# benedikthoward/ENPH459-Super-Resolution

Measured on AMD Instinct MI355X. Metric: HR megapixels/sec at x4 upscale (SAA + 80-iteration IBP reconstruction), higher is better.
Workload: dtype f32; 1 GPU; C2: x4 multi-frame SR of 64x64 LR patches -> 256x256 HR, N=16 frames (all 4x4 sub-pixel phases), 7x7 Gaussian PSF, shift_and_add + ibp(80 it, step 0.5); patches_per_gpu=1024, global_patches=1024, factor=4, frames=16, n_iter=80, parallelism=patch-sharded x1, no collective

## Files before the change

### enph459-super-resolution_amd/csrc/srx_dtile.hpp

```cpp
#pragma once
#include "srx_patch.hpp"

namespace srx {
namespace dtile {

using patch::AxisC;
using patch::AxisW;
using patch::f8;
using patch::FIX;
using patch::ld4;
using patch::ld_u2;
using patch::NN_PAD;
using patch::RW;
using patch::sload8;
using patch::SLOT0;
using patch::SLOT1;
using patch::st4;
using patch::u32x4;
using patch::YW;

constexpr int RY = 256;
constexpr int HL = 32;
constexpr int ALIGN_Y = 4, ALIGN_X = 16;

template <int NSX> struct Lds {
    static constexpr int NW = 4 * NSX;
    static constexpr int OFF_YT = NW * RW, OFF_YL = OFF_YT + 4 * YW, OFF_GT = OFF_YL + 4 * YW, OFF_GL = OFF_GT + 3 * YW,
                         OFF_ROW = OFF_GL + 3 * YW, OFF_PART = OFF_ROW + 256, WORDS = OFF_PART + 2 * NW + 2;
    static_assert(WORDS * 4 <= 160 * 1024, "LDS budget");
};

struct TileD {
    int oy, ox;
    int y0, y1, x0, x1;
    int ntab;
    int flags;
};

struct DArgs {
    int H, W, tiles_x, tiles_y;
    AxisC y, x;
    int ngrp, c01;
    float sn;
};

struct DTabs {
    const float *Mt;
    const unsigned *Mt8;
    const int *m8;
    const float *Ct;
    const AxisW *aw;
    const TileD *tiles;
    const unsigned long long *rowm, *colm;
    const int *nn;
    const uint2 *nrec;
    const uint2 *nent;
    const float2 *Mn;
    int ntabs;
    const float *k2;
};

struct AxisTiles {
    int n;
    int o[64], a[65];
};

static inline bool plan_axis_tiles(int L, int RL, int align, AxisTiles &at)
{
    if (L < RL || L % align)
// ... 270 lines not shown
#pragma unroll
            for (int i = 0; i < NW; i++)
                t += part[i];
            err_prev[(size_t)b * err_stride] = (t + Vtot[b]) * scale;
        }
        __syncthreads();
    }
    const int sq0 = ((td.oy + 64 * s) >> 2) * W * 16;
    const int tb0 = (((td.ox + 64 * u) >> 2) * H + td.oy + 64 * s) * 16;
    const int m80 = (((td.ox + 64 * u) >> 4) * H + td.oy + 64 * s) * 16;
    auto uniform64 = [](unsigned long long v) {
        return (unsigned long long)(unsigned)__builtin_amdgcn_readfirstlane((int)(unsigned)v) |
               (unsigned long long)(unsigned)__builtin_amdgcn_readfirstlane((int)(unsigned)(v >> 32)) << 32;
    };
    const unsigned long long rmask = C01 ? uniform64(tb.rowm[(size_t)((td.flags >> 8) & 0xfff) * 4 + s]) : 0ull;
    const unsigned long long cmask = C01 ? uniform64(tb.colm[(size_t)((td.flags >> 20) & 0xfff) * 4 + u]) : 0ull;

#define SRX_DT_LOCALS()                                              \
    int tid = tid0;                                                  \
    asm volatile("" : "+v"(tid));                                    \
    const int lane = tid & 63;                                       \
    int sql = sq0, tbl = tb0, m8l = m80;                             \
    asm volatile("" : "+s"(sql), "+s"(tbl), "+s"(m8l));              \
    const int vcol = (td.ox + 64 * u + lane) * 16;                   \
    (void)tbl, (void)m8l, (void)sql, (void)vcol

    float a[64], r[64];
    float yex = 0.f;
    {
        SRX_DT_LOCALS();
#pragma unroll
        for (int q = 0; q < 16; q++)
            ld4(rs_src, vcol, sql + q * W * 16, a[4 * q], a[4 * q + 1], a[4 * q + 2], a[4 * q + 3]);
        if (PSF == 0) {
            patch::blur_block(a, s == 0, s == 3, Rown, Rup, Rdn, SLOT0, lane, sload8(awy));
        } else {
            Rown[SLOT0 + lane] = a[0];
            Rown[SLOT0 + 64 + lane] = a[1];
            Rown[SLOT0 + 128 + lane] = a[2];
            Rown[SLOT0 + 192 + lane] = a[61];
            Rown[SLOT0 + 256 + lane] = a[62];
            Rown[SLOT0 + 320 + lane] = a[63];
            __syncthreads();
            float hl[3] = {0.f, 0.f, 0.f}, hr[3] = {0.f, 0.f, 0.f};
            if (s != 0)
                hl[0] = Rup[SLOT0 + 192 + lane], hl[1] = Rup[SLOT0 + 256 + lane], hl[2] = Rup[SLOT0 + 320 + lane];
            if (s != 3)
                hr[0] = Rdn[SLOT0 + lane], hr[1] = Rdn[SLOT0 + 64 + lane], hr[2] = Rdn[SLOT0 + 128 + lane];
            patch::blur2d_pass1<PSF == 2 ? 2 : 3>(a, hl, hr, Rown, lane, tb.k2);
            __syncthreads();
            patch::blur2d_fix<PSF == 2 ? 2 : 3>(a, u == 0, u == NSX - 1, Rown, Rlf, Rrt, lane, [](int) {}, [](int, float v) { return v; });
        }
        __builtin_amdgcn_sched_barrier(0);
        patch::fwd_chain(a, s == 0, s == 3, Rown, Rup, Rdn, SLOT1, SLOT0, lane, sload8(awy + 16), yex);
        __builtin_amdgcn_sched_barrier(0);
        if (exy && s == 0)
            rowbuf[64 * u + lane] = yex;
        __syncthreads();
        if (exy && s == 3)
            a[63] = rowbuf[64 * u + lane];
        __builtin_amdgcn_sched_barrier(0);
        patch::transpose64(a, r, Rown, lane);
        __builtin_amdgcn_sched_barrier(0);
    }
    float sq = 0.f;
    {
        SRX_DT_LOCALS();
        const bool wrapped = exy && s == 3 && lane == 63;
        const int gy = wrapped ? -1 : 64 * s + lane;
        const bool rownear = wrapped || gy < nby;
        const bool rowown = !wrapped && gy >= td.y0 && gy < td.y1;
        const float crow = C01 ? (float)((rmask >> lane) & 1ull) : 0.f;
        if (PSF == 0)
            patch::blur_block(r, u == 0, u == NSX - 1, Rown, Rlf, Rrt, SLOT0, lane, sload8(awx));
        __builtin_amdgcn_sched_barrier(0);
        float yexx = 0.f;
        patch::fwd_chain(r, u == 0, u == NSX - 1, Rown, Rlf, Rrt, SLOT1, SLOT0, lane, sload8(awx + 16), yexx);
        __builtin_amdgcn_sched_barrier(0);
        const __amdgpu_buffer_rsrc_t rsNe = fused::plane_rsrc(tb.nent, (size_t)da.ngrp * tb.ntabs * NN_PAD);
        const int tab0 = max(td.ntab, 0) * NN_PAD;
        if (nn > 0) {
            const __amdgpu_buffer_rsrc_t rsNr = fused::plane_rsrc(tb.nrec + tab0, (size_t)nn);
            const __amdgpu_buffer_rsrc_t rsMn = fused::plane_rsrc(tb.Mn + ((size_t)b * tb.ntabs) * NN_PAD + tab0, (size_t)nn);
            uint2 nr[NPT], ne[NPT];
            float2 nm[NPT];
#pragma unroll
            for (int i = 0; i < NPT; i++) {
                const int t8 = (tid + i * NTHR) * 8;
                nr[i] = ld_u2(rsNr, t8), ne[i] = ld_u2(rsNe, tab0 * 8 + t8);
                const uint2 m = ld_u2(rsMn, t8);
                nm[i] = make_float2(__uint_as_float(m.x), __uint_as_float(m.y));
            }
            {
                const bool toprow = wrapped || (s == 0 && lane <= nby);
                if (toprow) {
                    float *dst = Yt + (gy + exy) * YW + 64 * u + exx;
#pragma unroll
                    for (int j = 0; j < 64; j++)
                        dst[j] = r[j];
                    if (u == 0 && exx)
                        dst[-1] = yexx;
                }
                if (left && u == 0) {
                    float *dst = Yl + (gy + exy) * 4 + exx;
#pragma unroll
                    for (int j = 0; j < 3; j++)
                        if (j <= nbx)
                            dst[j] = r[j];
                    if (exx)
                        dst[-1] = yexx;
                }
            }
            __syncthreads();
#pragma unroll
            for (int i = 0; i < NPT; i++) {
                const int t = tid + i * NTHR;
                if (t < nn) {
                    const int cnt = nr[i].x & 255, cu = (nr[i].x >> 8) & 255, dst = nr[i].x >> 16;
                    float ys = (cnt > 0 ? Ystrip[ne[i].x & 0xffff] : 0.f) + (cnt > 1 ? Ystrip[ne[i].x >> 16] : 0.f) +
                               (cnt > 2 ? Ystrip[ne[i].y & 0xffff] : 0.f) + (cnt > 3 ? Ystrip[ne[i].y >> 16] : 0.f);
                    for (int g = 1; 4 * g < cnt; g++) {
                        const uint2 e = ld_u2(rsNe, ((g * tb.ntabs) * NN_PAD + tab0 + t) * 8);
                        const int c = cnt - 4 * g;
                        ys += (c > 0 ? Ystrip[e.x & 0xffff] : 0.f) + (c > 1 ? Ystrip[e.x >> 16] : 0.f) + (c > 2 ? Ystrip[e.y & 0xffff] : 0.f) +
                              (c > 3 ? Ystrip[e.y >> 16] : 0.f);
                    }
                    Gstrip[dst] = nm[i].x - ys;
                    if (cu > 0) {
                        const float gu = nm[i].y - (float)cu * Ystrip[nr[i].y];
                        sq += gu * gu / (float)cu;
// ... 113 lines not shown
            sq += (rownear || !rowown) ? 0.f : sqf;
            if ((top && s == 0) || (exy && s == 3)) {
                const float *src = Gt + (rownear ? gy + exy : 0) * YW + 64 * u + exx;
#pragma unroll
                for (int j0 = 0; j0 < 64; j0 += 8) {
                    float v[8];
                    int o = j0;
                    asm volatile("" : "+v"(o), "+v"(r[j0 > 0 ? j0 - 1 : 0])::"memory");
#pragma unroll
                    for (int j = 0; j < 8; j++)
                        v[j] = src[o + j];
#pragma unroll
                    for (int j = 0; j < 8; j++) {
                        r[j0 + j] = rownear ? v[j] : r[j0 + j];
                        asm volatile("" : "+v"(r[j0 + j]));
                    }
                    __builtin_amdgcn_sched_barrier(0);
                }
                if (u == 0 && exx && rownear)
                    gexx = src[-1];
            }
            if (left && u == 0 && !rownear) {
                const float *src = Gl + (gy - nby) * 3 + exx;
#pragma unroll
                for (int j = 0; j < 3; j++)
                    if (j < nbx)
                        r[j] = src[j];
                if (exx)
                    gexx = src[-1];
            }
        }
        if (epart) {
            const double ws = wave_sum((double)sq);
            if (lane == 0)
                part[wave] = ws;
        }
        __builtin_amdgcn_sched_barrier(0);
        {
            Rown[SLOT1 + lane] = r[0];
            Rown[SLOT1 + 64 + lane] = r[1];
            Rown[SLOT1 + 128 + lane] = r[63];
            __syncthreads();
            if (epart && tid == 0) {
                double t = 0.0;
#pragma unroll
                for (int i = 0; i < NW; i++)
                    t += part[i];
                epart[(size_t)b * gridDim.x + wid] = t;
            }
            const float gtop = exx ? gexx : r[0];
            const float gm1 = u == 0 ? gtop : Rlf[SLOT1 + 128 + lane];
            const float gp1 = u == NSX - 1 ? 0.f : Rrt[SLOT1 + lane], gp2 = u == NSX - 1 ? 0.f : Rrt[SLOT1 + 64 + lane];
            float hlo[3], hhi[3];
            patch::bwd_chain_x<PSF == 0>(r, a, u == 0, u == NSX - 1, Rown, Rlf, Rrt, SLOT0 + 384, SLOT0, lane, sload8(awx + 16), sload8(awx + 8), gm1, gp1, gp2, gtop,
                                         [](int) {}, [](int, float v) { return v; }, hlo, hhi);
        }
        __builtin_amdgcn_sched_barrier(0);
        __syncthreads();
        __builtin_amdgcn_sched_barrier(0);
        patch::transpose64(a, r, Rown, lane);
        __builtin_amdgcn_sched_barrier(0);
    }
    {
        SRX_DT_LOCALS();
        float hv[16], hw[16];
        if (exy && s == 3) {
            rowbuf[64 * u + lane] = r[63];
            r[63] = 0.f;
        }
        Rown[SLOT0 + lane] = r[0];
        Rown[SLOT0 + 64 + lane] = r[1];
        Rown[SLOT0 + 128 + lane] = r[63];
        __syncthreads();
        const float gtop = exy ? rowbuf[64 * u + lane] : r[0];
        const float gm1 = s == 0 ? gtop : Rup[SLOT0 + 128 + lane];
        const float gp1 = s == 3 ? 0.f : Rdn[SLOT0 + lane], gp2 = s == 3 ? 0.f : Rdn[SLOT0 + 64 + lane];
        float dep = 0.f;
        auto mid = [&](int q) {
                             auto load16 = [&](float(&ld)[16], int bq) {
                                 int so = sq0;
                                 asm volatile("" : "+s"(so), "+v"(dep)::"memory");
#pragma unroll
                                 for (int k = 0; k < 4; k++)
                                     ld4(rs_src, vcol, so + (4 * bq + k) * W * 16, ld[4 * k], ld[4 * k + 1], ld[4 * k + 2], ld[4 * k + 3]);
                             };
                             if (q == 0)
                                 load16(hv, 0), load16(hw, 1);
                             if (q == 1)
                                 load16(hv, 2);
                             else if (q == 2)
                                 load16(hw, 3);
                         };
        auto post = [&](int i, float corr) {
                             const float v = __builtin_amdgcn_fmed3f(fmaf(corr, sn, ((i >> 4) & 1) ? hw[i & 15] : hv[i & 15]), 0.f, 255.f);
                             if ((i & 15) == 15)
                                 dep = v;
                             return v;
                         };
        if (PSF == 0) {
            patch::bwd_chain(r, a, s == 0, s == 3, Rown, Rup, Rdn, SLOT1 + 384, SLOT1, lane, sload8(awy + 16), sload8(awy + 8), gm1, gp1, gp2, gtop, mid, post);
        } else {
            float hl[3], hr[3];
            patch::bwd_chain_x<false>(r, a, s == 0, s == 3, Rown, Rup, Rdn, SLOT1 + 384, SLOT1, lane, sload8(awy + 16), sload8(awy + 8), gm1, gp1, gp2, gtop, [](int) {},
                                      [](int, float v) { return v; }, hl, hr);
            patch::blur2d_pass1<PSF == 2 ? 2 : 3>(a, hl, hr, Rown, lane, tb.k2 + 56);
            __syncthreads();
            patch::blur2d_fix<PSF == 2 ? 2 : 3>(a, u == 0, u == NSX - 1, Rown, Rlf, Rrt, lane, mid, post);
        }
        __builtin_amdgcn_sched_barrier(0);
        const int cc = 64 * u + lane;
        const int vst = (cc >= td.x0 && cc < td.x1) ? vcol : 0x7ffffff0;
#pragma unroll
        for (int q = 0; q < 16; q++) {
            const int rw = 64 * s + 4 * q;
            if (rw >= td.y0 && rw < td.y1)
                st4(rs_dst, vst, sql + q * W * 16, a[4 * q], a[4 * q + 1], a[4 * q + 2], a[4 * q + 3]);
        }
    }
#undef SRX_DT_LOCALS
}

template <bool C01, int NSX, int PSF = 0>
__global__ void __launch_bounds__(256 * NSX)
    k_ibp_dtile(const float *__restrict__ hr_src, float *__restrict__ hr_dst, DTabs tb, DArgs da, double *__restrict__ epart,
                const double *__restrict__ eprev, const double *__restrict__ Vtot, double scale, double *__restrict__ err_prev, int err_stride)
{
    __shared__ float lds[Lds<NSX>::WORDS];
    if (__builtin_amdgcn_readfirstlane(tb.m8[blockIdx.y]) != 0)
        dtile_body<C01, true, NSX, PSF>(lds, hr_src, hr_dst, tb, da, epart, eprev, Vtot, scale, err_prev, err_stride);
    else
        dtile_body<C01, false, NSX, PSF>(lds, hr_src, hr_dst, tb, da, epart, eprev, Vtot, scale, err_prev, err_stride);
}

static inline size_t tabs_bytes(int B, int N, int H, int W)
{
    const size_t ngrp = ((size_t)N + 3) / 4, plane = (size_t)H * W, ntabs = 128, ntiles = 1024;
    return 3 * align_up((size_t)B * plane * 4) + align_up((size_t)B * (W / 4) * H * 4) + align_up((size_t)B * 4) + align_up(plane * 4) +
           align_up(2 * sizeof(AxisW)) + align_up(ntiles * sizeof(TileD)) + 2 * align_up(64 * 4 * 8) + align_up(ntabs * 4) +
           align_up(ntabs * NN_PAD * 8) + align_up(ngrp * ntabs * NN_PAD * 8) + align_up((size_t)B * ntabs * NN_PAD * 8) +
           2 * align_up((size_t)B * ntiles * 8) + align_up(112 * 4);
}

struct FrameN {
    int n[SRX_MAX_FRAMES];
};
__global__ void __launch_bounds__(256)
    k_dtile_setup(AxisTiles ty, AxisTiles tx, FrameN ny, FrameN nx, int N, int f, int H, int W, int nsx, TileD *__restrict__ tiles,
                  unsigned long long *__restrict__ rowm, unsigned long long *__restrict__ colm)
{
    const int tid = blockIdx.x * 256 + threadIdx.x;
    for (int i = tid; i < ty.n * tx.n; i += gridDim.x * 256) {
        const int y = i / tx.n, x = i - y * tx.n;
        TileD t;
        t.oy = ty.o[y], t.ox = tx.o[x];
        t.y0 = ty.a[y] - t.oy, t.y1 = ty.a[y + 1] - t.oy, t.x0 = tx.a[x] - t.ox, t.x1 = tx.a[x + 1] - t.ox;
        t.flags = (y == 0 ? 1 : 0) | (x == 0 ? 2 : 0) | y << 8 | x << 20;
// ... 137 lines not shown
```

### enph459-super-resolution_amd/csrc/srx_patch.hpp

```cpp
#pragma once
#include "srx_mosaic.hpp"

namespace srx {
namespace patch {

#ifndef SRX_PARK16
#define SRX_PARK16 1
#endif
#ifndef SRX_ADDTID
#define SRX_ADDTID 1
#endif
#ifndef SRX_M0_NOP
#define SRX_M0_NOP "s_nop 0\n\t"
#endif
#ifndef SRX_TRANSPOSE_DEF
#define SRX_TRANSPOSE_DEF 1
#endif
#ifndef SRX_PATCH_DBG
#define SRX_PATCH_DBG 0
#endif
constexpr int PN = 256;
constexpr int TSD = 66;
constexpr int RW = 32 * TSD;
constexpr int SLOT0 = 0, SLOT1 = 1024;
constexpr int FIX = 16;
constexpr int YW = 260;
constexpr int OFF_YT = 16 * RW, OFF_YL = OFF_YT + 4 * YW, OFF_GT = OFF_YL + 4 * YW, OFF_GL = OFF_GT + 3 * YW,
              OFF_ROW = OFF_GL + 3 * YW, OFF_PART = OFF_ROW + PN, LDS_WORDS = OFF_PART + 32;
static_assert(LDS_WORDS * 4 <= 160 * 1024, "LDS budget");

constexpr double ZD = -0.26794919243112270647;
constexpr float PZ = (float)ZD;
constexpr float K2 = (float)(1.0 / (1.0 - ZD));
constexpr float K1 = (float)(1.0 / ((1.0 - ZD) * (1.0 - ZD)));
constexpr float K3 = (float)(ZD / (1.0 - ZD * ZD));
constexpr float K4 = (float)(1.0 / (1.0 - ZD * ZD));
struct ZPow {
    float v[FIX];
    constexpr ZPow() : v()
    {
        double p = ZD;
        for (int i = 0; i < FIX; i++) {
            v[i] = (float)p;
            p *= ZD;
        }
    }
};
__device__ constexpr ZPow ZP{};

typedef float f8 __attribute__((ext_vector_type(8)));
struct AxisW {
    float kb[8];
    float kt[8];
    float wfb[8];
};
struct AxisC {
    int ex;
    int nb;
    int E;
};
__device__ __forceinline__ f8 sload8(const float *p)
{
    f8 v;
    asm volatile("s_load_dwordx8 %0, %1, 0x0\n\ts_waitcnt lgkmcnt(0)" : "=s"(v) : "s"(p) : "memory");
    return v;
}

constexpr int NN_PAD = 2048;

struct PatchArgs {
    AxisC y, x;
    int nn, ntop;
    int ngrp;
    int c01;
    unsigned long long ry[4], rx[4];
    float sn;
};

struct PatchTabs {
    const float *Mt;
    const unsigned *Mt8;
    const int *m8;
    const float *Ct;
    const AxisW *aw;
    const uint2 *nrec;
    const uint2 *nent;
    const float2 *Mn;
    const float *k2;
};

static inline bool axis_ok(const mosaic::AxisPlan &pl, int N, int f)
{
    int nmin = pl.n[0], nmax = pl.n[0];
    for (int k = 1; k < N; k++)
        nmin = std::min(nmin, pl.n[k]), nmax = std::max(nmax, pl.n[k]);
    return !pl.zero && nmax >= 0 && nmax <= 1 && nmin <= 0 && nmax - nmin <= 3 && nmax - nmin <= f - 1 && -nmin < f;
}

static inline bool eligible(int elem_bytes, int N, int H, int W, const double *sh, const double *k, int kh, int kw, int f, bool rank1_only)
{
    if (elem_bytes != 4 || H != PN || W != PN || f < 2)
// ... 294 lines not shown
                asm volatile("" : "=v"(r[j]));
        }
        if ((lane >> 5) == h) {
#else
        if (h == 0 || (lane >> 5) == h) {
#endif
            const float2 *row = reinterpret_cast<const float2 *>(Tw + (lane & 31) * TSD);
#pragma unroll
            for (int k = 0; k < 32; k++) {
                const float2 v = row[k];
                r[2 * k] = v.x, r[2 * k + 1] = v.y;
            }
        }
        __builtin_amdgcn_wave_barrier();
    }
}

#ifndef SRX_CHAIN_NSUB
#define SRX_CHAIN_NSUB 2
#endif
template <bool REV> __device__ __forceinline__ void chain64(float (&a)[64], float st0)
{
    constexpr int NSUB = SRX_CHAIN_NSUB, L = 64 / NSUB;
    static_assert(NSUB == 1 || L >= FIX, "a fix-up may not reach into the next sub-chain's start");
    const float z = PZ;
    auto at = [&](int i) -> float & { return a[REV ? 63 - i : i]; };
    float st[NSUB];
#pragma unroll
    for (int k = 0; k < NSUB; k++)
        st[k] = k == 0 ? st0 : 0.f;
#pragma unroll
    for (int i = 0; i < L; i++) {
#pragma unroll
        for (int k = 0; k < NSUB; k++) {
            st[k] = fmaf(z, st[k], at(k * L + i));
            at(k * L + i) = st[k];
        }
    }
    if (NSUB > 1) {
        float e[NSUB];
        e[0] = st[0];
#pragma unroll
        for (int k = 1; k < NSUB; k++)
            e[k] = L == FIX ? fmaf(ZP.v[FIX - 1], e[k - 1], st[k]) : st[k];
#pragma unroll
        for (int k = 1; k < NSUB; k++) {
#pragma unroll
            for (int i = 0; i < FIX; i++)
                at(k * L + i) = fmaf(ZP.v[i], e[k - 1], at(k * L + i));
        }
    }
}

__device__ __forceinline__ void fwd_chain(float (&a)[64], bool first, bool last, float *Rown, const float *Rprev, const float *Rnext,
                                          int sa, int sb, int lane, const f8 wfb, float &yex)
{
    const float z = PZ;
    const float bfirst = a[0], blast = a[63];
    chain64<false>(a, first ? bfirst * K2 : 0.f);
    Rown[sa + lane] = a[63];
    __syncthreads();
    if (!first) {
        const float carry = Rprev[sa + lane];
#pragma unroll
        for (int i = 0; i < FIX; i++)
            a[i] = fmaf(ZP.v[i], carry, a[i]);
    }
    const float cb = last ? fmaf(a[63] - blast * K2, K3, blast * K1) : 0.f;
    chain64<true>(a, cb);
    float cm1 = 0.f, cm2 = 0.f;
    if (first) {
        const float qs = bfirst * K2;
        cm1 = fmaf(z, a[0], qs);
        cm2 = fmaf(z, cm1, qs);
        const float cm3 = fmaf(z, cm2, qs);
        yex = wfb[0] * cm3 + wfb[1] * cm2 + wfb[2] * cm1 + wfb[3] * a[0];
    }
    Rown[sb + lane] = a[0];
    Rown[sb + 64 + lane] = a[62];
    Rown[sb + 128 + lane] = a[63];
    __syncthreads();
    float hb = cb;
    if (!last) {
        hb = Rnext[sb + lane];
#pragma unroll
        for (int i = 0; i < FIX; i++)
            a[63 - i] = fmaf(ZP.v[i], hb, a[63 - i]);
    }
    if (!first) {
        cm2 = fmaf(ZP.v[1], a[0], Rprev[sb + 64 + lane]);
        cm1 = fmaf(ZP.v[0], a[0], Rprev[sb + 128 + lane]);
    }
    float c2 = cm2, c1 = cm1;
#pragma unroll
    for (int i = 0; i < 64; i++) {
        const float c0 = a[i], cn = i < 63 ? a[i + 1] : hb;
        a[i] = wfb[0] * c2 + wfb[1] * c1 + wfb[2] * c0 + wfb[3] * cn;
        c2 = c1, c1 = c0;
    }
}

template <bool BLUR, typename F, typename P>
__device__ __forceinline__ void bwd_chain_x(float (&a)[64], float (&out)[64], bool first, bool last, float *Rown, const float *Rprev,
                                            const float *Rnext, int s1, int s6, int lane, const f8 wfb, const f8 kt, float gm1, float gp1,
                                            float gp2, float gtop, F mid, P post, float (&hlo)[3], float (&hhi)[3])
{
    const float z = PZ;
    const float w0 = wfb[4], w1 = wfb[5], w2 = wfb[6], w3 = wfb[7];
    const float vn = last ? w0 * a[63] : 0.f;
    SRX_PSTAMP(15);
    float st = 0.f;
    if (first) {
        st = (w0 + w1 + w2 + w3) * gtop * K2;
        st = fmaf(z, st, (w0 + w1 + w2) * gtop + w3 * a[0]);
        st = fmaf(z, st, (w0 + w1) * gtop + w2 * a[0] + w3 * a[1]);
    }
    float gprev = gm1;
#pragma unroll
    for (int t = 0; t < 64; t++) {
        const float g0 = a[t], g1 = t < 63 ? a[t + 1] : gp1, g2 = t < 62 ? a[t + 2] : (t == 62 ? gp1 : gp2);
        a[t] = w0 * gprev + w1 * g0 + w2 * g1 + w3 * g2;
        gprev = g0;
    }
    chain64<false>(a, st);
    SRX_PSTAMP(16);
    Rown[s1 + lane] = a[63];
    __syncthreads();
    SRX_PSTAMP(17);
    if (!first) {
        const float carry = Rprev[s1 + lane];
#pragma unroll
        for (int i = 0; i < FIX; i++)
            a[i] = fmaf(ZP.v[i], carry, a[i]);
    }
    const float cb = last ? fmaf(z, a[63], vn) * K4 : 0.f;
    chain64<true>(a, cb);
    Rown[s6 + lane] = a[0];
    Rown[s6 + 64 + lane] = a[1];
    Rown[s6 + 128 + lane] = a[2];
    Rown[s6 + 192 + lane] = a[61];
    Rown[s6 + 256 + lane] = a[62];
    Rown[s6 + 320 + lane] = a[63];
    SRX_PSTAMP(18);
    __syncthreads();
    SRX_PSTAMP(19);
    float e[70];
    e[0] = e[1] = e[2] = e[67] = e[68] = e[69] = 0.f;
    if (!last) {
        const float cn = Rnext[s6 + lane];
#pragma unroll
        for (int i = 0; i < FIX; i++)
            a[63 - i] = fmaf(ZP.v[i], cn, a[63 - i]);
        e[67] = cn, e[68] = Rnext[s6 + 64 + lane], e[69] = Rnext[s6 + 128 + lane];
    }
    if (!first) {
        e[0] = fmaf(ZP.v[2], a[0], Rprev[s6 + 192 + lane]);
        e[1] = fmaf(ZP.v[1], a[0], Rprev[s6 + 256 + lane]);
        e[2] = fmaf(ZP.v[0], a[0], Rprev[s6 + 320 + lane]);
    }
#pragma unroll
    for (int i = 0; i < 64; i++)
        e[3 + i] = a[i];
    SRX_PSTAMP(20);
    if (!BLUR) {
        hlo[0] = e[0], hlo[1] = e[1], hlo[2] = e[2], hhi[0] = e[67], hhi[1] = e[68], hhi[2] = e[69];
#pragma unroll
        for (int i = 0; i < 64; i++)
            out[i] = e[3 + i];
        return;
    }
#pragma unroll
    for (int q = 0; q < 4; q++) {
        mid(q);
#pragma unroll
        for (int i = 16 * q; i < 16 * q + 16; i++) {
            float acc = kt[0] * e[i];
#pragma unroll
            for (int u = 1; u < 7; u++)
                acc = fmaf(kt[u], e[i + u], acc);
            out[i] = post(i, acc);
        }
        __builtin_amdgcn_sched_barrier(0);
    }
}

template <typename F, typename P>
__device__ __forceinline__ void bwd_chain(float (&a)[64], float (&out)[64], bool first, bool last, float *Rown, const float *Rprev,
                                          const float *Rnext, int s1, int s6, int lane, const f8 wfb, const f8 kt, float gm1, float gp1,
                                          float gp2, float gtop, F mid, P post)
{
    float hlo[3], hhi[3];
    bwd_chain_x<true>(a, out, first, last, Rown, Rprev, Rnext, s1, s6, lane, wfb, kt, gm1, gp1, gp2, gtop, mid, post, hlo, hhi);
}

__device__ __forceinline__ void blur_block(float (&a)[64], bool first, bool last, float *Rown, const float *Rprev, const float *Rnext,
                                           int s6, int lane, const f8 kb)
{
    Rown[s6 + lane] = a[0];
    Rown[s6 + 64 + lane] = a[1];
    Rown[s6 + 128 + lane] = a[2];
    Rown[s6 + 192 + lane] = a[61];
    Rown[s6 + 256 + lane] = a[62];
    Rown[s6 + 320 + lane] = a[63];
    __syncthreads();
    float hl[3] = {0.f, 0.f, 0.f}, hr[3] = {0.f, 0.f, 0.f};
    if (!first)
        hl[0] = Rprev[s6 + 192 + lane], hl[1] = Rprev[s6 + 256 + lane], hl[2] = Rprev[s6 + 320 + lane];
    if (!last)
        hr[0] = Rnext[s6 + lane], hr[1] = Rnext[s6 + 64 + lane], hr[2] = Rnext[s6 + 128 + lane];
    float c0 = hl[0], c1 = hl[1], c2 = hl[2];
#pragma unroll
    for (int j0 = 0; j0 < 64; j0 += 8) {
        float w[14];
        w[0] = c0, w[1] = c1, w[2] = c2;
#pragma unroll
        for (int j = 0; j < 8; j++)
            w[3 + j] = a[j0 + j];
#pragma unroll
        for (int j = 0; j < 3; j++)
            w[11 + j] = j0 + 8 + j < 64 ? a[j0 + 8 + j] : hr[j];
        c0 = w[8], c1 = w[9], c2 = w[10];
#pragma unroll
        for (int j = 0; j < 8; j++) {
            float acc = kb[0] * w[j];
#pragma unroll
            for (int k = 1; k < 7; k++)
                acc = fmaf(kb[k], w[j + k], acc);
            a[j0 + j] = acc;
        }
        __builtin_amdgcn_sched_barrier(0);
    }
}

typedef float f2 __attribute__((ext_vector_type(2)));
typedef float f4 __attribute__((ext_vector_type(4)));
__device__ __forceinline__ float lane_up(float v) { return __int_as_float(__builtin_amdgcn_update_dpp(0, __float_as_int(v), 0x138, 0xf, 0xf, true)); }
__device__ __forceinline__ float lane_dn(float v) { return __int_as_float(__builtin_amdgcn_update_dpp(0, __float_as_int(v), 0x130, 0xf, 0xf, true)); }
constexpr int SLOT_E = 1536;
constexpr int SLOT_D = 512;
constexpr int SLOT_Z = 2048;
static_assert(SLOT_D >= SLOT0 + 448 && SLOT_D + 256 <= SLOT1 && SLOT_E >= SLOT1 + 448 && SLOT_E + 512 <= SLOT_Z && SLOT_Z + 8 <= RW, "slots inside the wave's region");

#ifndef SRX_PATCH_B2D_NB
#define SRX_PATCH_B2D_NB 4
#endif
// ... 125 lines not shown
    const int park0 = wave * 16384;
#endif
    for (int it = 0; it < n_iter; it++) {
        float r[64];
#define SRX_STAGE_LOCALS()                                 \
    int tid = tid0;                                        \
    asm volatile("" : "+v"(tid));                          \
    const int lane = tid & 63, l4 = lane * 4;              \
    int cbl = cb0, tbl = tb0, m8l = (4 * u * PN + 64 * s) * 16; \
    asm volatile("" : "+s"(cbl), "+s"(tbl), "+s"(m8l));    \
    (void)tbl, (void)m8l, (void)cbl, (void)l4
        float yex = 0.f;
        {
        SRX_STAGE_LOCALS();
        __builtin_amdgcn_sched_barrier(0);
        SRX_PSTAMP(0);
        if (!(SRX_PATCH_DBG & 8)) {
#if SRX_PARK16
            int pk = park0;
            asm volatile("" : "+s"(pk));
#pragma unroll
            for (int q = 0; q < 16; q++)
                st4(rs_out, l4 * 4, pk + q * 1024, a[4 * q], a[4 * q + 1], a[4 * q + 2], a[4 * q + 3]);
#else
#pragma unroll
            for (int i = 0; i < 64; i++)
                fused::buf_store<float>(a[i], rs_out, l4 + (i & 3) * PN * 4, cbl + (i >> 2) * PN * 16);
#endif
        }
        if (PSF == 0) {
            blur_block(a, s == 0, s == 3, Rown, Rup, Rdn, SLOT0, lane, sload8(awy));
        } else {
            Rown[SLOT0 + lane] = a[0];
            Rown[SLOT0 + 64 + lane] = a[1];
            Rown[SLOT0 + 128 + lane] = a[2];
            Rown[SLOT0 + 192 + lane] = a[61];
            Rown[SLOT0 + 256 + lane] = a[62];
            Rown[SLOT0 + 320 + lane] = a[63];
            __syncthreads();
            float hl[3] = {0.f, 0.f, 0.f}, hr[3] = {0.f, 0.f, 0.f};
            if (s != 0)
                hl[0] = Rup[SLOT0 + 192 + lane], hl[1] = Rup[SLOT0 + 256 + lane], hl[2] = Rup[SLOT0 + 320 + lane];
            if (s != 3)
                hr[0] = Rdn[SLOT0 + lane], hr[1] = Rdn[SLOT0 + 64 + lane], hr[2] = Rdn[SLOT0 + 128 + lane];
            blur2d_pass1<PSF == 2 ? 2 : 3>(a, hl, hr, Rown, lane, tb.k2);
            __syncthreads();
            blur2d_fix<PSF == 2 ? 2 : 3>(a, u == 0, u == 3, Rown, Rlf, Rrt, lane, [](int) {}, [](int, float v) { return v; });
#ifdef SRX_PATCH_B2D_SYNC
            __syncthreads();
#endif
        }
        __builtin_amdgcn_sched_barrier(0);
        SRX_PSTAMP(1);
        fwd_chain(a, s == 0, s == 3, Rown, Rup, Rdn, SLOT1, SLOT0, lane, sload8(awy + 16), yex);
        __builtin_amdgcn_sched_barrier(0);
        SRX_PSTAMP(2);
        if (exy && s == 0)
            rowbuf[64 * u + lane] = yex;
        __syncthreads();
        if (exy && s == 3)
            a[63] = rowbuf[64 * u + lane];
        __builtin_amdgcn_sched_barrier(0);
        SRX_PSTAMP(3);
        transpose64(a, r, Rown, lane);
        __builtin_amdgcn_sched_barrier(0);
        SRX_PSTAMP(4);
        }
        float sq = 0.f;
        {
        SRX_STAGE_LOCALS();
        const bool wrapped = exy && s == 3 && lane == 63;
        const int gy = wrapped ? -1 : 64 * s + lane;
        const bool rownear = wrapped || gy < nby;
        const float crow = C01 ? (float)((rmask >> lane) & 1ull) : 0.f;
        if (PSF == 0)
            blur_block(r, u == 0, u == 3, Rown, Rlf, Rrt, SLOT0, lane, sload8(awx));
        __builtin_amdgcn_sched_barrier(0);
        __builtin_amdgcn_sched_barrier(0);
        SRX_PSTAMP(5);
        float yexx = 0.f;
        fwd_chain(r, u == 0, u == 3, Rown, Rlf, Rrt, SLOT1, SLOT0, lane, sload8(awx + 16), yexx);
        __builtin_amdgcn_sched_barrier(0);
        SRX_PSTAMP(6);
        uint2 nr0 = make_uint2(0, 0), nr1 = make_uint2(0, 0), ne0 = make_uint2(0, 0), ne1 = make_uint2(0, 0);
        float2 nm0 = make_float2(0.f, 0.f), nm1 = make_float2(0.f, 0.f);
        const bool n0 = tid < nn, n1 = tid + 1024 < nn;
        const __amdgpu_buffer_rsrc_t rsNr = fused::plane_rsrc(tb.nrec, (size_t)nn), rsNe = fused::plane_rsrc(tb.nent, (size_t)pa.ngrp * NN_PAD),
                                     rsMn = fused::plane_rsrc(tb.Mn + (size_t)b * NN_PAD, (size_t)nn);
        {
            const int t8 = tid * 8;
            nr0 = ld_u2(rsNr, t8), ne0 = ld_u2(rsNe, t8);
            nr1 = ld_u2(rsNr, t8 + 8192), ne1 = ld_u2(rsNe, t8 + 8192);
            const uint2 m0 = ld_u2(rsMn, t8), m1 = ld_u2(rsMn, t8 + 8192);
            nm0 = make_float2(__uint_as_float(m0.x), __uint_as_float(m0.y)), nm1 = make_float2(__uint_as_float(m1.x), __uint_as_float(m1.y));
        }
        {
            const bool toprow = wrapped || (s == 0 && lane <= nby);
            if (toprow) {
                float *dst = Yt + (gy + exy) * YW + 64 * u + exx;
#pragma unroll
                for (int j = 0; j < 64; j++)
                    dst[j] = r[j];
                if (u == 0 && exx)
                    dst[-1] = yexx;
            }
            if (u == 0) {
                float *dst = Yl + (gy + exy) * 4 + exx;
#pragma unroll
                for (int j = 0; j < 3; j++)
                    if (j <= nbx)
                        dst[j] = r[j];
                if (exx)
                    dst[-1] = yexx;
            }
        }
        __syncthreads();
        const __amdgpu_buffer_rsrc_t rsM8 = fused::plane_rsrc(tb.Mt8 + (size_t)b * (PN / 4) * PN, (size_t)(PN / 4) * PN);
        unsigned m8w[16];
        if (m8) {
#pragma unroll
            for (int q = 0; q < 4; q++) {
                const u32x4 v = (SRX_PATCH_DBG & 1) ? u32x4{0x01020304u, 0x01020304u, 0x01020304u, 0x01020304u}
                                                    : __builtin_amdgcn_raw_buffer_load_b128(rsM8, l4 * 4, m8l + q * PN * 16, 0);
                m8w[4 * q] = v.x, m8w[4 * q + 1] = v.y, m8w[4 * q + 2] = v.z, m8w[4 * q + 3] = v.w;
            }
        }
        __builtin_amdgcn_sched_barrier(0);
        SRX_PSTAMP(7);
        {
            auto near_px = [&](uint2 nr, uint2 ne, float2 nm, int t) {
                const int cnt = nr.x & 255, cu = (nr.x >> 8) & 255, dst = nr.x >> 16;
                float ys = (cnt > 0 ? Ystrip[ne.x & 0xffff] : 0.f) + (cnt > 1 ? Ystrip[ne.x >> 16] : 0.f) +
                           (cnt > 2 ? Ystrip[ne.y & 0xffff] : 0.f) + (cnt > 3 ? Ystrip[ne.y >> 16] : 0.f);
                for (int g = 1; 4 * g < cnt; g++) {
// ... 66 lines not shown
                    for (int j = 0; j < 16; j++) {
                        const float g = fmaf(-cv[j], r[j0 + j], mv[j]);
                        const float g2 = g * g * (C01 ? 1.f : mosaic::rcp_count(cv[j]));
                        sqf += g2;
                        if (j0 + j < 3)
                            gn[j0 + j] = g2;
                        r[j0 + j] = g;
                    }
                }
            }
            if (u == 0)
                sqf -= (nbx > 0 ? gn[0] : 0.f) + (nbx > 1 ? gn[1] : 0.f) + (nbx > 2 ? gn[2] : 0.f);
            sq += (rownear || (SRX_PATCH_DBG & 32)) ? 0.f : sqf;
            if (rownear) {
                const float *src = Gt + (gy + exy) * YW + 64 * u + exx;
#pragma unroll
                for (int j = 0; j < 64; j++)
                    r[j] = src[j];
                if (u == 0 && exx)
                    gexx = src[-1];
            } else if (u == 0) {
                const float *src = Gl + (gy - nby) * 3 + exx;
#pragma unroll
                for (int j = 0; j < 3; j++)
                    if (j < nbx)
                        r[j] = src[j];
                if (exx)
                    gexx = src[-1];
            }
        }
        if (errors) {
            const double ws = wave_sum((double)sq);
            if (lane == 0)
                part[wave] = ws;
        }
        __builtin_amdgcn_sched_barrier(0);
        SRX_PSTAMP(9);
        {
            Rown[SLOT1 + lane] = r[0];
            Rown[SLOT1 + 64 + lane] = r[1];
            Rown[SLOT1 + 128 + lane] = r[63];
            __syncthreads();
            if (errors && tid == 0) {
                double t = 0.0;
#pragma unroll
                for (int i = 0; i < 16; i++)
                    t += part[i];
                errors[(size_t)b * n_iter + it] = (t + Vtot[b]) * scale;
            }
            const float gtop = exx ? gexx : r[0];
            const float gm1 = u == 0 ? gtop : Rlf[SLOT1 + 128 + lane];
            const float gp1 = u == 3 ? 0.f : Rrt[SLOT1 + lane], gp2 = u == 3 ? 0.f : Rrt[SLOT1 + 64 + lane];
            float hlo[3], hhi[3];
            bwd_chain_x<PSF == 0>(r, a, u == 0, u == 3, Rown, Rlf, Rrt, SLOT0 + 384, SLOT0, lane, sload8(awx + 16), sload8(awx + 8), gm1, gp1, gp2, gtop, [](int) {},
                                  [](int, float v) { return v; }, hlo, hhi);
        }
        __builtin_amdgcn_sched_barrier(0);
        SRX_PSTAMP(10);
        __syncthreads();
        __builtin_amdgcn_sched_barrier(0);
        SRX_PSTAMP(11);
        transpose64(a, r, Rown, lane);
        __builtin_amdgcn_sched_barrier(0);
        SRX_PSTAMP(12);
        }
        {
        SRX_STAGE_LOCALS();
        float hv[16], hw[16];
        {
            if (exy && s == 3) {
                rowbuf[64 * u + lane] = r[63];
                r[63] = 0.f;
            }
            Rown[SLOT0 + lane] = r[0];
            Rown[SLOT0 + 64 + lane] = r[1];
            Rown[SLOT0 + 128 + lane] = r[63];
            __syncthreads();
            const float gtop = exy ? rowbuf[64 * u + lane] : r[0];
            const float gm1 = s == 0 ? gtop : Rup[SLOT0 + 128 + lane];
            const float gp1 = s == 3 ? 0.f : Rdn[SLOT0 + lane], gp2 = s == 3 ? 0.f : Rdn[SLOT0 + 64 + lane];
            auto mid = [&](int q) {
                          auto load16 = [&](float(&ld)[16], int bq) {
#if SRX_PARK16
                              int pk = park0;
                              asm volatile("" : "+s"(pk));
#pragma unroll
                              for (int q = 0; q < 4; q++) {
                                  if (SRX_PATCH_DBG & 2)
                                      ld[4 * q] = ld[4 * q + 1] = ld[4 * q + 2] = ld[4 * q + 3] = 1.f;
                                  else
                                      ld4(rs_out, l4 * 4, pk + (4 * bq + q) * 1024, ld[4 * q], ld[4 * q + 1], ld[4 * q + 2], ld[4 * q + 3]);
                              }
#else
#pragma unroll
                              for (int i = 0; i < 16; i++)
                                  ld[i] = (SRX_PATCH_DBG & 2) ? 1.f : fused::buf_load<float>(rs_out, l4 + (i & 3) * PN * 4, cbl + (4 * bq + (i >> 2)) * PN * 16);
#endif
                          };
                          if (q == 0) {
                              SRX_PSTAMP(13);
                              load16(hv, 0), load16(hw, 1);
                          }
                          if (q == 1)
                              load16(hv, 2);
                          else if (q == 2)
                              load16(hw, 3);
                      };
            auto post = [&](int i, float corr) {
                          return __builtin_amdgcn_fmed3f(fmaf(corr, sn, ((i >> 4) & 1) ? hw[i & 15] : hv[i & 15]), 0.f, 255.f);
                      };
            if (PSF == 0) {
                bwd_chain(r, a, s == 0, s == 3, Rown, Rup, Rdn, SLOT1 + 384, SLOT1, lane, sload8(awy + 16), sload8(awy + 8), gm1, gp1, gp2, gtop, mid, post);
            } else {
                float hl[3], hr[3];
                bwd_chain_x<false>(r, a, s == 0, s == 3, Rown, Rup, Rdn, SLOT1 + 384, SLOT1, lane, sload8(awy + 16), sload8(awy + 8), gm1, gp1, gp2, gtop, [](int) {},
                                   [](int, float v) { return v; }, hl, hr);
                blur2d_pass1<PSF == 2 ? 2 : 3>(a, hl, hr, Rown, lane, tb.k2 + 56);
                __syncthreads();
                blur2d_fix<PSF == 2 ? 2 : 3>(a, u == 0, u == 3, Rown, Rlf, Rrt, lane, mid, post);
#ifdef SRX_PATCH_B2D_SYNC
                __syncthreads();
#endif
            }
        }
        __builtin_amdgcn_sched_barrier(0);
        SRX_PSTAMP(14);
        }
#undef SRX_STAGE_LOCALS
    }
    {
#if SRX_PARK16
        asm volatile("s_waitcnt vmcnt(0)" ::: "memory");
        __syncthreads();
#endif
        const int l4 = (tid0 & 63) * 4;
#pragma unroll
        for (int i = 0; i < 64; i++)
            fused::buf_store<float>(a[i], rs_out, l4 + (i & 3) * PN * 4, cb0 + (i >> 2) * PN * 16);
    }
}

static inline void fill_axis(const mosaic::AxisPlan &pl, int N, const float *cfwd, const float *cbwd, AxisC &ax, AxisW &aw)
{
    const double kq = -6.0 * ZD;
    int nmin = pl.n[0], nmax = pl.n[0];
    for (int k = 1; k < N; k++)
        nmin = std::min(nmin, pl.n[k]), nmax = std::max(nmax, pl.n[k]);
    double wv[4];
    fused::host_weights(1.0 - pl.delta, wv);
    for (int i = 0; i < 4; i++)
        aw.wfb[i] = (float)wv[i];
    fused::host_weights(pl.delta, wv);
    for (int i = 0; i < 4; i++)
        aw.wfb[4 + i] = (float)(kq * wv[i]);
    aw.kb[7] = aw.kt[7] = 0.f;
    for (int i = 0; i < 7; i++)
        aw.kb[i] = (float)(kq * (double)cfwd[i]), aw.kt[i] = cbwd[i];
    ax.ex = nmax, ax.nb = -nmin, ax.E = pl.E;
}

static inline bool c01_masks(const mosaic::AxisPlan &py, const mosaic::AxisPlan &px, int N, int f, unsigned long long ry[4],
                             unsigned long long rx[4])
{
    int ny[SRX_MAX_FRAMES], nx[SRX_MAX_FRAMES], cy = 0, cx = 0;
    for (int k = 0; k < N; k++) {
        bool fy = false, fx = false;
        for (int j = 0; j < cy; j++)
            fy = fy || ny[j] == py.n[k];
// ... 190 lines not shown
```

Before: 5568 HR-MP/s.

## Merge forward/backward recursive-filter carry exchanges into one barrier in dtile path

Adds a ONEX mode to the forward and backward recursive chain helpers. It removes the mid-chain __syncthreads after the causal pass and defers the incoming carry correction until after the single remaining barrier. Precomputed alpha coefficients (ZAlpha) fold the causal carry's effect into the anticausal boundary values algebraically. The dtile kernel uses ONEX=true with a new LDS slot for the forward chain, while the patch kernel keeps the old two-barrier path. The cost is extra FMAs and LDS reads, plus reliance on the truncated FIX-term approximation of the carry propagation.

```diff
diff --git a/enph459-super-resolution_amd/csrc/srx_dtile.hpp b/enph459-super-resolution_amd/csrc/srx_dtile.hpp
--- a/enph459-super-resolution_amd/csrc/srx_dtile.hpp
+++ b/enph459-super-resolution_amd/csrc/srx_dtile.hpp
@@ -15,6 +15,7 @@
 using patch::sload8;
 using patch::SLOT0;
 using patch::SLOT1;
+using patch::SLOT_F;
 using patch::st4;
 using patch::u32x4;
 using patch::YW;
@@ -391,7 +392,7 @@
             patch::blur2d_fix<PSF == 2 ? 2 : 3>(a, u == 0, u == NSX - 1, Rown, Rlf, Rrt, lane, [](int) {}, [](int, float v) { return v; });
         }
         __builtin_amdgcn_sched_barrier(0);
-        patch::fwd_chain(a, s == 0, s == 3, Rown, Rup, Rdn, SLOT1, SLOT0, lane, sload8(awy + 16), yex);
+        patch::fwd_chain<true>(a, s == 0, s == 3, Rown, Rup, Rdn, SLOT_F, SLOT_F + 64, lane, sload8(awy + 16), yex);
         __builtin_amdgcn_sched_barrier(0);
         if (exy && s == 0)
             rowbuf[64 * u + lane] = yex;
@@ -414,7 +415,7 @@
             patch::blur_block(r, u == 0, u == NSX - 1, Rown, Rlf, Rrt, SLOT0, lane, sload8(awx));
         __builtin_amdgcn_sched_barrier(0);
         float yexx = 0.f;
-        patch::fwd_chain(r, u == 0, u == NSX - 1, Rown, Rlf, Rrt, SLOT1, SLOT0, lane, sload8(awx + 16), yexx);
+        patch::fwd_chain<true>(r, u == 0, u == NSX - 1, Rown, Rlf, Rrt, SLOT_F, SLOT_F + 64, lane, sload8(awx + 16), yexx);
         __builtin_amdgcn_sched_barrier(0);
         const __amdgpu_buffer_rsrc_t rsNe = fused::plane_rsrc(tb.nent, (size_t)da.ngrp * tb.ntabs * NN_PAD);
         const int tab0 = max(td.ntab, 0) * NN_PAD;
@@ -634,7 +635,7 @@
             const float gm1 = u == 0 ? gtop : Rlf[SLOT1 + 128 + lane];
             const float gp1 = u == NSX - 1 ? 0.f : Rrt[SLOT1 + lane], gp2 = u == NSX - 1 ? 0.f : Rrt[SLOT1 + 64 + lane];
             float hlo[3], hhi[3];
-            patch::bwd_chain_x<PSF == 0>(r, a, u == 0, u == NSX - 1, Rown, Rlf, Rrt, SLOT0 + 384, SLOT0, lane, sload8(awx + 16), sload8(awx + 8), gm1, gp1, gp2, gtop,
+            patch::bwd_chain_x<PSF == 0, true>(r, a, u == 0, u == NSX - 1, Rown, Rlf, Rrt, SLOT0 + 384, SLOT0, lane, sload8(awx + 16), sload8(awx + 8), gm1, gp1, gp2, gtop,
                                          [](int) {}, [](int, float v) { return v; }, hlo, hhi);
         }
         __builtin_amdgcn_sched_barrier(0);
@@ -680,10 +681,10 @@
                              return v;
                          };
         if (PSF == 0) {
-            patch::bwd_chain(r, a, s == 0, s == 3, Rown, Rup, Rdn, SLOT1 + 384, SLOT1, lane, sload8(awy + 16), sload8(awy + 8), gm1, gp1, gp2, gtop, mid, post);
+            patch::bwd_chain<true>(r, a, s == 0, s == 3, Rown, Rup, Rdn, SLOT1 + 384, SLOT1, lane, sload8(awy + 16), sload8(awy + 8), gm1, gp1, gp2, gtop, mid, post);
         } else {
             float hl[3], hr[3];
-            patch::bwd_chain_x<false>(r, a, s == 0, s == 3, Rown, Rup, Rdn, SLOT1 + 384, SLOT1, lane, sload8(awy + 16), sload8(awy + 8), gm1, gp1, gp2, gtop, [](int) {},
+            patch::bwd_chain_x<false, true>(r, a, s == 0, s == 3, Rown, Rup, Rdn, SLOT1 + 384, SLOT1, lane, sload8(awy + 16), sload8(awy + 8), gm1, gp1, gp2, gtop, [](int) {},
                                       [](int, float v) { return v; }, hl, hr);
             patch::blur2d_pass1<PSF == 2 ? 2 : 3>(a, hl, hr, Rown, lane, tb.k2 + 56);
             __syncthreads();
diff --git a/enph459-super-resolution_amd/csrc/srx_patch.hpp b/enph459-super-resolution_amd/csrc/srx_patch.hpp
--- a/enph459-super-resolution_amd/csrc/srx_patch.hpp
+++ b/enph459-super-resolution_amd/csrc/srx_patch.hpp
@@ -23,6 +23,8 @@
 constexpr int TSD = 66;
 constexpr int RW = 32 * TSD;
 constexpr int SLOT0 = 0, SLOT1 = 1024;
+constexpr int SLOT_F = SLOT1 + 192;
+static_assert(SLOT_F >= SLOT1 + 192 && SLOT_F + 256 <= SLOT1 + 448, "forward-chain slot inside SLOT1's 7 x 64 words");
 constexpr int FIX = 16;
 constexpr int YW = 260;
 constexpr int OFF_YT = 16 * RW, OFF_YL = OFF_YT + 4 * YW, OFF_GT = OFF_YL + 4 * YW, OFF_GL = OFF_GT + 3 * YW,
@@ -47,6 +49,21 @@
     }
 };
 __device__ constexpr ZPow ZP{};
+struct ZAlpha {
+    float v[FIX];
+    constexpr ZAlpha() : v()
+    {
+        for (int i = 0; i < FIX; i++) {
+            double p = ZD, s = 0.0, q = 1.0;
+            for (int k = 0; k < i; k++)
+                p *= ZD;
+            for (int m = 0; m < FIX - i; m++, q *= ZD * ZD)
+                s += q;
+            v[i] = (float)(p * s);
+        }
+    }
+};
+__device__ constexpr ZAlpha AL{};
 
 typedef float f8 __attribute__((ext_vector_type(8)));
 struct AxisW {
@@ -447,6 +464,7 @@
     }
 }
 
+template <bool ONEX>
 __device__ __forceinline__ void fwd_chain(float (&a)[64], bool first, bool last, float *Rown, const float *Rprev, const float *Rnext,
                                           int sa, int sb, int lane, const f8 wfb, float &yex)
 {
@@ -454,12 +472,14 @@
     const float bfirst = a[0], blast = a[63];
     chain64<false>(a, first ? bfirst * K2 : 0.f);
     Rown[sa + lane] = a[63];
-    __syncthreads();
-    if (!first) {
-        const float carry = Rprev[sa + lane];
-#pragma unroll
-        for (int i = 0; i < FIX; i++)
-            a[i] = fmaf(ZP.v[i], carry, a[i]);
+    if (!ONEX) {
+        __syncthreads();
+        if (!first) {
+            const float carry = Rprev[sa + lane];
+#pragma unroll
+            for (int i = 0; i < FIX; i++)
+                a[i] = fmaf(ZP.v[i], carry, a[i]);
+        }
     }
     const float cb = last ? fmaf(a[63] - blast * K2, K3, blast * K1) : 0.f;
     chain64<true>(a, cb);
@@ -475,9 +495,17 @@
     Rown[sb + 64 + lane] = a[62];
     Rown[sb + 128 + lane] = a[63];
     __syncthreads();
+    if (ONEX && !first) {
+        const float carry = Rprev[sa + lane];
+#pragma unroll
+        for (int i = 0; i < FIX; i++)
+            a[i] = fmaf(AL.v[i], carry, a[i]);
+    }
     float hb = cb;
     if (!last) {
         hb = Rnext[sb + lane];
+        if (ONEX)
+            hb = fmaf(AL.v[0], Rown[sa + lane], hb);
 #pragma unroll
         for (int i = 0; i < FIX; i++)
             a[63 - i] = fmaf(ZP.v[i], hb, a[63 - i]);
@@ -495,7 +523,7 @@
     }
 }
 
-template <bool BLUR, typename F, typename P>
+template <bool BLUR, bool ONEX, typename F, typename P>
 __device__ __forceinline__ void bwd_chain_x(float (&a)[64], float (&out)[64], bool first, bool last, float *Rown, const float *Rprev,
                                             const float *Rnext, int s1, int s6, int lane, const f8 wfb, const f8 kt, float gm1, float gp1,
                                             float gp2, float gtop, F mid, P post, float (&hlo)[3], float (&hhi)[3])
@@ -520,13 +548,15 @@
     chain64<false>(a, st);
     SRX_PSTAMP(16);
     Rown[s1 + lane] = a[63];
-    __syncthreads();
-    SRX_PSTAMP(17);
-    if (!first) {
-        const float carry = Rprev[s1 + lane];
-#pragma unroll
-        for (int i = 0; i < FIX; i++)
-            a[i] = fmaf(ZP.v[i], carry, a[i]);
+    if (!ONEX) {
+        __syncthreads();
+        SRX_PSTAMP(17);
+        if (!first) {
+            const float carry = Rprev[s1 + lane];
+#pragma unroll
+            for (int i = 0; i < FIX; i++)
+                a[i] = fmaf(ZP.v[i], carry, a[i]);
+        }
     }
     const float cb = last ? fmaf(z, a[63], vn) * K4 : 0.f;
     chain64<true>(a, cb);
@@ -541,12 +571,22 @@
     SRX_PSTAMP(19);
     float e[70];
     e[0] = e[1] = e[2] = e[67] = e[68] = e[69] = 0.f;
+    if (ONEX && !first) {
+        const float carry = Rprev[s1 + lane];
+#pragma unroll
+        for (int i = 0; i < FIX; i++)
+            a[i] = fmaf(AL.v[i], carry, a[i]);
+    }
     if (!last) {
-        const float cn = Rnext[s6 + lane];
+        float cn = Rnext[s6 + lane], cn1 = Rnext[s6 + 64 + lane], cn2 = Rnext[s6 + 128 + lane];
+        if (ONEX) {
+            const float E = Rown[s1 + lane];
+            cn = fmaf(AL.v[0], E, cn), cn1 = fmaf(AL.v[1], E, cn1), cn2 = fmaf(AL.v[2], E, cn2);
+        }
 #pragma unroll
         for (int i = 0; i < FIX; i++)
             a[63 - i] = fmaf(ZP.v[i], cn, a[63 - i]);
-        e[67] = cn, e[68] = Rnext[s6 + 64 + lane], e[69] = Rnext[s6 + 128 + lane];
+        e[67] = cn, e[68] = cn1, e[69] = cn2;
     }
     if (!first) {
         e[0] = fmaf(ZP.v[2], a[0], Rprev[s6 + 192 + lane]);
@@ -579,13 +619,13 @@
     }
 }
 
-template <typename F, typename P>
+template <bool ONEX, typename F, typename P>
 __device__ __forceinline__ void bwd_chain(float (&a)[64], float (&out)[64], bool first, bool last, float *Rown, const float *Rprev,
                                           const float *Rnext, int s1, int s6, int lane, const f8 wfb, const f8 kt, float gm1, float gp1,
                                           float gp2, float gtop, F mid, P post)
 {
     float hlo[3], hhi[3];
-    bwd_chain_x<true>(a, out, first, last, Rown, Rprev, Rnext, s1, s6, lane, wfb, kt, gm1, gp1, gp2, gtop, mid, post, hlo, hhi);
+    bwd_chain_x<true, ONEX>(a, out, first, last, Rown, Rprev, Rnext, s1, s6, lane, wfb, kt, gm1, gp1, gp2, gtop, mid, post, hlo, hhi);
 }
 
 __device__ __forceinline__ void blur_block(float (&a)[64], bool first, bool last, float *Rown, const float *Rprev, const float *Rnext,
@@ -817,7 +857,7 @@
         }
         __builtin_amdgcn_sched_barrier(0);
         SRX_PSTAMP(1);
-        fwd_chain(a, s == 0, s == 3, Rown, Rup, Rdn, SLOT1, SLOT0, lane, sload8(awy + 16), yex);
+        fwd_chain<false>(a, s == 0, s == 3, Rown, Rup, Rdn, SLOT1, SLOT0, lane, sload8(awy + 16), yex);
         __builtin_amdgcn_sched_barrier(0);
         SRX_PSTAMP(2);
         if (exy && s == 0)
@@ -844,7 +884,7 @@
         __builtin_amdgcn_sched_barrier(0);
         SRX_PSTAMP(5);
         float yexx = 0.f;
-        fwd_chain(r, u == 0, u == 3, Rown, Rlf, Rrt, SLOT1, SLOT0, lane, sload8(awx + 16), yexx);
+        fwd_chain<false>(r, u == 0, u == 3, Rown, Rlf, Rrt, SLOT1, SLOT0, lane, sload8(awx + 16), yexx);
         __builtin_amdgcn_sched_barrier(0);
         SRX_PSTAMP(6);
         uint2 nr0 = make_uint2(0, 0), nr1 = make_uint2(0, 0), ne0 = make_uint2(0, 0), ne1 = make_uint2(0, 0);
@@ -1017,7 +1057,7 @@
             const float gm1 = u == 0 ? gtop : Rlf[SLOT1 + 128 + lane];
             const float gp1 = u == 3 ? 0.f : Rrt[SLOT1 + lane], gp2 = u == 3 ? 0.f : Rrt[SLOT1 + 64 + lane];
             float hlo[3], hhi[3];
-            bwd_chain_x<PSF == 0>(r, a, u == 0, u == 3, Rown, Rlf, Rrt, SLOT0 + 384, SLOT0, lane, sload8(awx + 16), sload8(awx + 8), gm1, gp1, gp2, gtop, [](int) {},
+            bwd_chain_x<PSF == 0, false>(r, a, u == 0, u == 3, Rown, Rlf, Rrt, SLOT0 + 384, SLOT0, lane, sload8(awx + 16), sload8(awx + 8), gm1, gp1, gp2, gtop, [](int) {},
                                   [](int, float v) { return v; }, hlo, hhi);
         }
         __builtin_amdgcn_sched_barrier(0);
@@ -1075,10 +1115,10 @@
                           return __builtin_amdgcn_fmed3f(fmaf(corr, sn, ((i >> 4) & 1) ? hw[i & 15] : hv[i & 15]), 0.f, 255.f);
                       };
             if (PSF == 0) {
-                bwd_chain(r, a, s == 0, s == 3, Rown, Rup, Rdn, SLOT1 + 384, SLOT1, lane, sload8(awy + 16), sload8(awy + 8), gm1, gp1, gp2, gtop, mid, post);
+                bwd_chain<false>(r, a, s == 0, s == 3, Rown, Rup, Rdn, SLOT1 + 384, SLOT1, lane, sload8(awy + 16), sload8(awy + 8), gm1, gp1, gp2, gtop, mid, post);
             } else {
                 float hl[3], hr[3];
-                bwd_chain_x<false>(r, a, s == 0, s == 3, Rown, Rup, Rdn, SLOT1 + 384, SLOT1, lane, sload8(awy + 16), sload8(awy + 8), gm1, gp1, gp2, gtop, [](int) {},
+                bwd_chain_x<false, false>(r, a, s == 0, s == 3, Rown, Rup, Rdn, SLOT1 + 384, SLOT1, lane, sload8(awy + 16), sload8(awy + 8), gm1, gp1, gp2, gtop, [](int) {},
                                    [](int, float v) { return v; }, hl, hr);
                 blur2d_pass1<PSF == 2 ? 2 : 3>(a, hl, hr, Rown, lane, tb.k2 + 56);
                 __syncthreads();
```

Measured after the change: 5573 HR-MP/s, median of 6. No clear change (+0.1%).
